# apache/bifromq

Hardware: AMD Instinct MI355X
Metric: publish-topic matches/sec (whole node) (higher is better)
Workload: dtype u32

## Files before the change

bifromq_amd/csrc/bmq_expand_kernel.h:

```cpp
#pragma once

namespace bmq {

constexpr uint32_t SORT_PAIRS = 32;
#ifndef BMQ_EXP_K
#define BMQ_EXP_K 256
#endif
#ifndef BMQ_EXP_LONG
#define BMQ_EXP_LONG 64
#endif
#ifndef BMQ_EXP_CLOCKS
#define BMQ_EXP_CLOCKS 0
#endif
#ifndef BMQ_EXP_MIN_WAVES
#define BMQ_EXP_MIN_WAVES 6
#endif
constexpr uint32_t EXP_K = BMQ_EXP_K;
constexpr uint32_t EXP_LONG = BMQ_EXP_LONG;
constexpr uint32_t EXP_EPL = EXP_K / 64;
constexpr uint32_t EXP_FLAG_WORDS = (EXP_K * (EXP_LONG - 1) + 63) / 64 + 2;
static_assert(EXP_K % 64 == 0 && EXP_K >= 2 * SORT_PAIRS && EXP_K * (EXP_LONG - 1) < 65536, "short-range space: sums are packed into 16 bits below");

#ifndef BMQ_WAVE_EMU
__device__ __forceinline__ uint32_t read_lane(uint32_t v, uint32_t l) { return __builtin_amdgcn_readlane(v, l); }
template <int CTRL, int ROWS> __device__ __forceinline__ uint32_t dpp_take(uint32_t v) {
    return (uint32_t)__builtin_amdgcn_update_dpp(0, (int)v, CTRL, ROWS, 0xF, false);
}
__device__ __forceinline__ uint32_t lane_bit(unsigned long long m) { return (uint32_t)(m >> threadIdx.x) & 1u; }
__device__ __forceinline__ uint32_t first_bit(unsigned long long m) { return (uint32_t)__ffsll((long long)m) - 1u; }
__device__ __forceinline__ uint32_t count_bits(unsigned long long m) { return (uint32_t)__popcll(m); }
__device__ __forceinline__ uint32_t copy_here(uint32_t v) {
    uint32_t r;
    asm volatile("v_mov_b32 %0, %1" : "=v"(r) : "v"(v));
    return r;
}
__device__ __forceinline__ uint32_t uniform_word(const uint32_t* p) { return *scalar_words(p); }
#endif
__device__ __forceinline__ unsigned long long sgpr64(unsigned long long v) {
    return ((unsigned long long)sgpr((uint32_t)(v >> 32)) << 32) | sgpr((uint32_t)v);
}
__device__ __forceinline__ uint32_t wave_incl_scan(uint32_t v) {
    v += dpp_take<0x111, 0xF>(v);
    v += dpp_take<0x112, 0xF>(v);
    v += dpp_take<0x114, 0xF>(v);
    v += dpp_take<0x118, 0xF>(v);
    v += dpp_take<0x142, 0xA>(v);
    v += dpp_take<0x143, 0xC>(v);
    return v;
}
template <int CTRL, int ROWS> __device__ __forceinline__ unsigned long long dpp_take64(unsigned long long v) {
    return ((unsigned long long)dpp_take<CTRL, ROWS>((uint32_t)(v >> 32)) << 32) | dpp_take<CTRL, ROWS>((uint32_t)v);
}
__device__ __forceinline__ unsigned long long wave_total_u64(unsigned long long v) {
    v += dpp_take64<0x111, 0xF>(v);
    v += dpp_take64<0x112, 0xF>(v);
    v += dpp_take64<0x114, 0xF>(v);
    v += dpp_take64<0x118, 0xF>(v);
    v += dpp_take64<0x142, 0xA>(v);
    v += dpp_take64<0x143, 0xC>(v);
    return ((unsigned long long)read_lane((uint32_t)(v >> 32), 63) << 32) | read_lane((uint32_t)v, 63);
}

__device__ __forceinline__ void expand_wave(const BatchArgs& a, const uint32_t block_x, const uint32_t r0 = 0u, const uint32_t r1 = 64u) {
    __shared__ uint32_t s_begin[EXP_K], s_cnt[EXP_K];
    __shared__ uint32_t s_delta[EXP_K + 4];
    __shared__ unsigned long long s_flag[EXP_FLAG_WORDS];
    __shared__ unsigned long long s_rs[2][EXP_EPL];
    __shared__ unsigned long long s_rows[1];
    __shared__ uint32_t s_ind[EXP_K / 32];
    __shared__ uint32_t l_po[64], l_px[65];
    __shared__ uint8_t nz[64];
    uint32_t* const s_key = s_delta;
    const uint32_t lane = threadIdx.x;
    const uint32_t blk = block_x;
    if (blk >= a.n_blocks) return;
    const uint32_t t = (blk << a.tpw_shift) + lane;
    const bool valid = lane < (1u << a.tpw_shift) && t < a.n_topics;
    const bool dbg_x = BMQ_EXP_CLOCKS && BMQ_DBG(a, 4u) && a.dbg_wave;
    const unsigned long long xc0 = dbg_x ? __builtin_amdgcn_s_memtime() : 0ull;
    unsigned long long xc_load = 0, xc_scan = 0, xc_gen = 0;
    const uint32_t status = uniform_word(&a.ctr->status);
    const uint32_t tt = valid ? t : 0u;
    uint32_t nr = a.route_cnt[tt], po = a.pair_off[tt], np = a.pair_cnt[tt];
    unsigned long long acc = 0;
    {
        const uint32_t sb = blk >> SUPER_SHIFT, w0 = sb << SUPER_SHIFT;
        const unsigned long long s0 = a.super_sums[(size_t)min(lane, sb) * SUPER_STRIDE];
        unsigned long long w[4];
#pragma unroll
        for (uint32_t j = 0; j < 4; j++) w[j] = a.wave_sums[min(w0 + lane + 64u * j, blk)];
        static_assert(SUPER_SHIFT == 8, "four loads per lane cover a super-block");
        for (uint32_t i = lane + 64u; i < sb; i += 64) acc += a.super_sums[(size_t)i * SUPER_STRIDE];
        if (lane < sb) acc += s0;
#pragma unroll
        for (uint32_t j = 0; j < 4; j++)
            if (w0 + lane + 64u * j < blk) acc += w[j];
    }
    if (!valid) nr = 0u, po = 0u, np = 0u;
    const bool mine = lane >= r0 && lane < r1;
    if (!mine) np = 0u;
    if (r0 == 0u && a.blk_stats && ((blk & ((1u << SUPER_SHIFT) - 1u)) == (1u << SUPER_SHIFT) - 1u || blk == a.n_blocks - 1)) {
        unsigned long long v = 0, r = 0, b = 0;
        for (uint32_t i = ((blk >> SUPER_SHIFT) << SUPER_SHIFT) + lane; i <= blk; i += 64) {
            const uint4 q = a.blk_stats[i];
            v += q.x, r += q.y, b += q.z;
        }
        v = wave_total_u64(v), r = wave_total_u64(r), b = wave_total_u64(b);
        if (lane == 0) {
            if (v) atomicAdd(&a.ctr->n_visit, v);
            if (r) atomicAdd(&a.ctr->n_ranges, r);
            if (b) atomicAdd(&a.ctr->topic_bytes, b);
        }
    }
    const uint32_t nr_incl = wave_incl_scan(nr);
    const uint32_t wtotal = read_lane(nr_incl, 63);
    const unsigned long long wbase = wave_total_u64(acc);
    const unsigned long long row = wbase + (nr_incl - nr);
    const unsigned long long wend = wbase + wtotal;
    const bool range_err = wend >= 0xFFFFFFFFull, no_space = wend > a.out_capacity;
    if (blk == a.n_blocks - 1 && lane == 0 && r0 == 0u) {
        a.ctr->total_ids = wend;
        *a.out_total = wend;
    }
    if ((range_err || no_space) && lane == 0) atomicOr(&a.ctr->status, range_err ? (uint32_t)ST_RANGE : (uint32_t)ST_NOSPACE);
    const bool writable = !(status & ST_RERUN) && !range_err && !no_space;
    if (valid && mine && !range_err) {
        a.out_row_ptr[t] = (uint32_t)row;
        if (t == a.n_topics - 1) a.out_row_ptr[a.n_topics] = (uint32_t)(row + nr);
    }
    if (!writable || wtotal == 0) return;
    const uint32_t np_incl = wave_incl_scan(np);
    const uint32_t ptotal = read_lane(np_incl, 63);
    if (ptotal == 0) return;
    const uint32_t pexcl = np_incl - np;
    const unsigned long long m_np = ballot64(np != 0);
    const uint32_t first_l = m_np ? first_bit(m_np) : 0u;
    const uint32_t po0 = read_lane(po, first_l) - read_lane(pexcl, first_l);
    const bool contiguous = ballot64(np != 0 && po != po0 + pexcl) == 0ull && !BMQ_DBG(a, 64u);
    l_po[lane] = po;
    l_px[lane] = pexcl;
    if (lane == 63) l_px[64] = ptotal;
    if (np) nz[rank_below(m_np)] = (uint8_t)lane;
    for (uint32_t i = lane; i < EXP_FLAG_WORDS; i += 64) s_flag[i] = 0ull;
    if (lane < EXP_K / 32) s_ind[lane] = 0u;
    if (lane == 0) s_rows[0] = 0ull;
    wave_sync();
    struct Pass {
        uint32_t kn;
        uint32_t ord0;
        uint32_t continues;
    };
    auto plan = [&](uint32_t k0, unsigned long long* rs) -> Pass {
        Pass p;
        p.kn = min(EXP_K, ptotal - k0);
        {
            const uint32_t kend = k0 + p.kn;
            const unsigned long long m = ballot64(pexcl < kend && kend < pexcl + np && np <= SORT_PAIRS);
            if (m) p.kn = read_lane(pexcl, first_bit(m)) - k0;
        }
        const uint32_t lo = pexcl > k0 ? pexcl : k0, hi = min(pexcl + np, k0 + p.kn);
        if (lane < EXP_EPL) rs[lane] = 0ull;
        wave_sync();
        if (lo < hi) atomicOr(&rs[(lo - k0) >> 6], 1ull << ((lo - k0) & 63u));
        const unsigned long long m_k0 = ballot64(np != 0 && pexcl <= k0 && k0 < pexcl + np);
        const uint32_t lk = first_bit(m_k0);
        p.ord0 = count_bits(m_np & ((1ull << lk) - 1ull));
        p.continues = read_lane(pexcl, lk) < k0 ? 1u : 0u;
        wave_sync();
        return p;
    };
    MatchRange pf[EXP_EPL];
    auto fetch = [&](uint32_t k0, const Pass& p, const unsigned long long* rs) {
        const uint32_t lane = lane_here();
        if (contiguous) {
#pragma unroll
            for (uint32_t i = 0; i < EXP_EPL; i++) pf[i] = a.pairs[po0 + k0 + min(lane + 64 * i, p.kn - 1u)];
        } else {
            uint32_t c = p.ord0 - 1u;
            uint32_t at[EXP_EPL];
            const uint32_t l0 = nz[p.ord0];
            const uint32_t at0 = l_po[l0] + (k0 - l_px[l0]);
#pragma unroll
            for (uint32_t i = 0; i < EXP_EPL; i++) {
                const unsigned long long w = sgpr64(rs[i]);
                const uint32_t e = lane + 64 * i;
                at[i] = at0;
                if (e < p.kn) {
                    const uint32_t l = nz[c + rank_below(w) + lane_bit(w)];
                    at[i] = l_po[l] + (k0 + e - l_px[l]);
                }
                c += count_bits(w);
            }
#pragma unroll
            for (uint32_t i = 0; i < EXP_EPL; i++) pf[i] = a.pairs[at[i]];
        }
    };
#pragma unroll
    for (uint32_t i = 0; i < EXP_EPL; i++) pf[i] = MatchRange{0u, 0u};
    Pass cur = plan(0u, s_rs[0]);
    fetch(0u, cur, s_rs[0]);
    uint32_t eb[EXP_EPL], ec[EXP_EPL];
    __builtin_amdgcn_s_waitcnt(0x0F70);
#pragma unroll
    for (uint32_t i = 0; i < EXP_EPL; i++) eb[i] = copy_here(pf[i].begin), ec[i] = copy_here(pf[i].count);
    const unsigned long long xc1 = dbg_x ? __builtin_amdgcn_s_memtime() : 0ull;
    uint32_t pass = 0;
    unsigned long long out_done = read_lane(nr_incl - nr, r0);
    uint32_t carry_last = 0;
    for (uint32_t k0 = 0; k0 < ptotal; pass++) {
        const unsigned long long xp0 = dbg_x ? __builtin_amdgcn_s_memtime() : 0ull;
        const uint32_t kn = cur.kn;
        const bool continues = cur.continues != 0u;
        const unsigned long long* rs = s_rs[pass & 1u];
        unsigned long long rsw[EXP_EPL];
        uint32_t rsc[EXP_EPL];
        {
            uint32_t c = cur.ord0 - 1u;
#pragma unroll
            for (uint32_t i = 0; i < EXP_EPL; i++) {
                rsw[i] = sgpr64(rs[i]);
                rsc[i] = c;
                c += count_bits(rsw[i]);
            }
        }
        unsigned long long m_ind = 0;
#pragma unroll
        for (uint32_t i = 0; i < EXP_EPL; i++) m_ind |= ballot64(lane + 64 * i < kn && (ec[i] & RANGE_INDIRECT) != 0u);
        const bool more = k0 + kn < ptotal;
        Pass nxt = cur;
        if (more) {
            nxt = plan(k0 + kn, s_rs[(pass + 1u) & 1u]);
            fetch(k0 + kn, nxt, s_rs[(pass + 1u) & 1u]);
        }
        auto body = [&](auto ind_tag) {
            constexpr bool IND = decltype(ind_tag)::value;
            auto first_id = [&](uint32_t b, uint32_t cf) -> uint32_t { return (IND && (cf & RANGE_INDIRECT)) ? a.ix.route_pos[b] : b; };
            auto last_id = [&](uint32_t b, uint32_t cf) -> uint32_t {
                const uint32_t c = cf & ~RANGE_INDIRECT;
                return (IND && (cf & RANGE_INDIRECT)) ? a.ix.route_pos[b + c - 1u] : b + c - 1u;
            };
            uint32_t ek[EXP_EPL];
#pragma unroll
            for (uint32_t i = 0; i < EXP_EPL; i++) {
                const uint32_t e = lane + 64 * i;
                ek[i] = eb[i];
                if (e < kn) {
                    ek[i] = first_id(eb[i], ec[i]);
                    s_begin[e] = eb[i];
                    s_cnt[e] = ec[i];
                    s_key[e] = ek[i];
                }
            }
            wave_sync();
            unsigned long long any_bad = 0;
#pragma unroll
            for (uint32_t i = 0; i < EXP_EPL; i++) {
                const uint32_t e = lane + 64 * i;
                bool bad = false;
                if (e < kn && (e == 0u ? continues : lane_bit(rsw[i]) == 0u)) {
                    const uint32_t plast = e == 0u ? carry_last : last_id(s_begin[e - 1u], s_cnt[e - 1u]);
                    bad = ek[i] <= plast;
                }
                any_bad |= ballot64(bad);
            }
            if (any_bad) {
                uint32_t to[EXP_EPL];
#pragma unroll
                for (uint32_t i = 0; i < EXP_EPL; i++) {
                    const uint32_t e = lane + 64 * i;
                    to[i] = e;
                    if (e < kn) {
                        const uint32_t l = nz[rsc[i] + rank_below(rsw[i]) + lane_bit(rsw[i])];
                        const uint32_t s0 = l_px[l], n = l_px[l + 1u] - s0;
                        if (n > 1u && n <= SORT_PAIRS) {
                            const uint32_t first = s0 - k0;
                            const unsigned long long mine = ((unsigned long long)ek[i] << 32) | e;
                            uint32_t rank = 0;
                            const uint32_t end = first + n;
#pragma nounroll
                            for (uint32_t j = first; j < end; j += 4) {
                                const uint32_t q0 = s_key[j], q1 = s_key[j + 1u], q2 = s_key[j + 2u], q3 = s_key[j + 3u];
                                rank += ((((unsigned long long)q0) << 32) | j) < mine ? 1u : 0u;
                                rank += (j + 1u < end && ((((unsigned long long)q1) << 32) | (j + 1u)) < mine) ? 1u : 0u;
                                rank += (j + 2u < end && ((((unsigned long long)q2) << 32) | (j + 2u)) < mine) ? 1u : 0u;
                                rank += (j + 3u < end && ((((unsigned long long)q3) << 32) | (j + 3u)) < mine) ? 1u : 0u;
                            }
                            to[i] = first + rank;
                        }
                    }
                }
                wave_sync();
#pragma unroll
                for (uint32_t i = 0; i < EXP_EPL; i++)
                    if (lane + 64 * i < kn) {
                        s_begin[to[i]] = eb[i];
                        s_cnt[to[i]] = ec[i];
                        s_key[to[i]] = ek[i];
                    }
                wave_sync();
#pragma unroll
                for (uint32_t i = 0; i < EXP_EPL; i++) {
                    const uint32_t e = lane + 64 * i;
                    if (e < kn && (e == 0u ? continues : lane_bit(rsw[i]) == 0u)) {
                        const uint32_t plast = e == 0u ? carry_last : last_id(s_begin[e - 1u], s_cnt[e - 1u]);
                        if (s_key[e] <= plast) {
                            const uint32_t l = nz[rsc[i] + rank_below(rsw[i]) + lane_bit(rsw[i])];
                            atomicOr(&s_rows[0], 1ull << l);
                        }
                    }
                }
            }
            carry_last = sgpr(last_id(s_begin[kn - 1u], s_cnt[kn - 1u]));
            wave_sync();
            const unsigned long long xp1 = dbg_x ? __builtin_amdgcn_s_memtime() : 0ull;
            uint32_t T, stot;
            {
                uint32_t pb[EXP_EPL], pc[EXP_EPL];
                uint32_t s = 0, ss = 0;
                const uint32_t e0 = lane * EXP_EPL;
#pragma unroll
                for (uint32_t i = 0; i < EXP_EPL; i++) {
                    const uint32_t e = e0 + i;
                    pb[i] = e < kn ? s_begin[e] : 0u;
                    pc[i] = e < kn ? s_cnt[e] : 0u;
                    const uint32_t len = pc[i] & ~RANGE_INDIRECT;
                    s += len;
                    if (len - 1u < EXP_LONG - 1u) ss += len + (1u << 16);
                }
                const uint32_t s_incl = wave_incl_scan(s), ss_incl = wave_incl_scan(ss);
                T = read_lane(s_incl, 63);
                stot = read_lane(ss_incl, 63);
                uint32_t run = s_incl - s;
                uint32_t us = (ss_incl - ss) & 0xFFFFu, ord = (ss_incl - ss) >> 16;
#pragma unroll
                for (uint32_t i = 0; i < EXP_EPL; i++) {
                    const uint32_t e = e0 + i;
                    if (e < kn) {
                        const uint32_t len = pc[i] & ~RANGE_INDIRECT;
                        if (len - 1u < EXP_LONG - 1u) {
                            s_delta[ord] = pb[i] - us;
                            if (IND && (pc[i] & RANGE_INDIRECT)) atomicOr(&s_ind[ord >> 5], 1u << (ord & 31u));
                            us += len;
                            atomicOr(&s_flag[(us - 1u) >> 6], 1ull << ((us - 1u) & 63u));
                            ord++;
                        } else s_delta[EXP_K - 1u - (e - ord)] = run;
                        run += len;
                    }
                }
            }
            wave_sync();
            const unsigned long long xp2 = dbg_x ? __builtin_amdgcn_s_memtime() : 0ull;
            __builtin_amdgcn_s_waitcnt(0x0F70);
#pragma unroll
            for (uint32_t i = 0; i < EXP_EPL; i++) eb[i] = copy_here(pf[i].begin), ec[i] = copy_here(pf[i].count);
            {
                uint32_t* const out = a.out_ids + wbase + out_done;
                const bool other = (stot >> 16) != kn;
                uint32_t outp = 0;
                uint32_t ub = 0;
                uint32_t lq = 0;
                uint32_t fw = 0, fo = 0;
                unsigned long long fm = sgpr64(s_flag[0]), fnext = sgpr64(s_flag[1]);
                for (uint32_t k = 0; k < kn;) {
                    uint32_t kl = kn;
                    if (other)
                        for (uint32_t c0 = k; c0 < kn && kl == kn; c0 += 64) {
                            const unsigned long long m = ballot64(c0 + lane < kn && (s_cnt[c0 + lane] & ~RANGE_INDIRECT) - 1u >= EXP_LONG - 1u);
                            if (m) kl = c0 + first_bit(m);
                        }
                    const uint32_t run_end = kl < kn ? sgpr(s_delta[EXP_K - 1u - lq]) : T;
                    if (run_end != outp) {
                        const uint32_t ue = ub + (run_end - outp);
                        uint32_t* const dst = out + outp;
                        for (uint32_t c = ub & ~63u; c < ue; c += 64) {
                            if (fw < (c >> 6)) {
                                fo += count_bits(fm);
                                fw++;
                                fm = fnext;
                                fnext = sgpr64(s_flag[min(fw + 1u, EXP_FLAG_WORDS - 1u)]);
                            }
                            const uint32_t u = c + lane;
                            if (u >= ub && u < ue) {
                                const uint32_t o = fo + rank_below(fm);
                                uint32_t v = s_delta[o] + u;
                                if (IND && ((s_ind[o >> 5] >> (o & 31u)) & 1u)) v = a.ix.route_pos[v];
                                dst[u - ub] = v;
                            }
                        }
                        ub = ue;
                    }
                    if (kl < kn) {
                        const uint32_t b = sgpr(s_begin[kl]), cf = sgpr(s_cnt[kl]), c = cf & ~RANGE_INDIRECT;
                        uint32_t* const dst = out + run_end;
                        if (IND && (cf & RANGE_INDIRECT)) {
                            for (uint32_t o = lane; o < c; o += 64) dst[o] = a.ix.route_pos[b + o];
                        } else {
                            const uint32_t head = min((uint32_t)(((16u - ((uintptr_t)dst & 15u)) & 15u) >> 2), c);
                            if (lane < head) dst[lane] = b + lane;
                            uint4* d4 = reinterpret_cast<uint4*>(dst + head);
                            const uint32_t n4 = (c - head) >> 2;
                            for (uint32_t q = lane; q < n4; q += 64) {
                                const uint32_t v = b + head + 4 * q;
                                d4[q] = make_uint4(v, v + 1, v + 2, v + 3);
                            }
                            for (uint32_t o = head + 4 * n4 + lane; o < c; o += 64) dst[o] = b + o;
                        }
                        outp = run_end + c;
                        lq++;
                    }
                    k = kl + 1;
                }
            }
            out_done += T;
            if (more) {
                wave_sync();
                for (uint32_t i = lane; i <= ((stot & 0xFFFFu) >> 6); i += 64) s_flag[i] = 0ull;
                if (IND && lane < EXP_K / 32 && lane <= (stot >> 21)) s_ind[lane] = 0u;
                wave_sync();
            }
            if (dbg_x) {
                const unsigned long long xp3 = __builtin_amdgcn_s_memtime();
                xc_load += xp1 - xp0, xc_scan += xp2 - xp1, xc_gen += xp3 - xp2;
            }
        };
        if (m_ind) body(std::true_type{});
        else body(std::false_type{});
        k0 += kn;
        cur = nxt;
    }
    if (dbg_x && lane == 0) a.dbg_wave[blk] = make_uint4((uint32_t)(xc1 - xc0), (uint32_t)xc_load, (uint32_t)xc_scan, (uint32_t)xc_gen);
    wave_sync();
    if (valid && lane_bit(s_rows[0]) && nr > 1) {
        const uint32_t sp = atomicAdd(&a.ctr->sort_count, 1u);
        if (sp < a.sort_cap) a.sort_list[sp] = t;
        else atomicOr(&a.ctr->status, ST_NEED_SORTLIST);
    }
}

__global__ __launch_bounds__(64, BMQ_EXP_MIN_WAVES) void k_expand(BatchArgs a) {
    uint32_t bx = blockIdx.x;
    if (a.heavy_list == nullptr) return expand_wave(a, bx);
    constexpr uint32_t HP = EXPAND_PARTS - 1u, RP = 64u / EXPAND_PARTS;
    const uint32_t n_help = HP * a.heavy_cap;
    if (bx < n_help) {
        const uint32_t listed = min(uniform_word(&a.ctr->heavy_count), a.heavy_cap);
        const uint32_t h = bx / HP, part = 1u + bx % HP;
        if (h >= listed) return;
        return expand_wave(a, uniform_word(&a.heavy_list[h]), part * RP, (part + 1u) * RP);
    }
    bx -= n_help;
    if (bx >= a.n_blocks) return;
    const bool split = uniform_word(reinterpret_cast<const uint32_t*>(a.blk_stats + bx) + 3) != 0u;
    expand_wave(a, bx, 0u, split ? RP : 64u);
}

}
```

Measured before the change: 3.994 billion.

## Compact sort to flagged groups and prefetch next flag-chunk delta lookups

After: 4.041 billion, median of 6. +1.2%, better.

```diff
diff --git a/bifromq_amd/csrc/bmq_expand_kernel.h b/bifromq_amd/csrc/bmq_expand_kernel.h
--- a/bifromq_amd/csrc/bmq_expand_kernel.h
+++ b/bifromq_amd/csrc/bmq_expand_kernel.h
@@ -20,6 +20,28 @@
 constexpr uint32_t EXP_EPL = EXP_K / 64;
 constexpr uint32_t EXP_FLAG_WORDS = (EXP_K * (EXP_LONG - 1) + 63) / 64 + 2;
 static_assert(EXP_K % 64 == 0 && EXP_K >= 2 * SORT_PAIRS && EXP_K * (EXP_LONG - 1) < 65536, "short-range space: sums are packed into 16 bits below");
+constexpr uint32_t EXP_IDX_BITS = EXP_K <= 256 ? 8u : 16u;
+using exp_idx_t = std::conditional_t<(EXP_K <= 256), uint16_t, uint32_t>;
+
+#ifdef BMQ_WAVE_EMU
+struct ExpandCoverage {
+    unsigned long long passes = 0, fast_passes = 0;
+    unsigned long long sort_passes = 0;
+    unsigned long long sort_entries = 0, sort_groups = 0;
+    unsigned long long groups[EXP_EPL + 1] = {};
+    unsigned long long unsortable = 0;
+    unsigned long long interleaved = 0;
+    unsigned long long carry_bad = 0;
+    unsigned long long chunks = 0, chunks_held = 0;
+    unsigned long long chunks_ahead = 0;
+};
+inline ExpandCoverage expand_cov;
+#define BMQ_EXP_COV(stmt) do { if (threadIdx.x == 0) { stmt; } } while (0)
+#define BMQ_EXP_COV_ANY(stmt) do { stmt; } while (0)
+#else
+#define BMQ_EXP_COV_ANY(stmt) do { } while (0)
+#define BMQ_EXP_COV(stmt) do { } while (0)
+#endif
 
 #ifndef BMQ_WAVE_EMU
 __device__ __forceinline__ uint32_t read_lane(uint32_t v, uint32_t l) { return __builtin_amdgcn_readlane(v, l); }
@@ -67,6 +89,8 @@
     __shared__ unsigned long long s_flag[EXP_FLAG_WORDS];
     __shared__ unsigned long long s_rs[2][EXP_EPL];
     __shared__ unsigned long long s_rows[1];
+    __shared__ unsigned long long s_need[1];
+    __shared__ exp_idx_t s_idx[EXP_K];
     __shared__ uint32_t s_ind[EXP_K / 32];
     __shared__ uint32_t l_po[64], l_px[65];
     __shared__ uint8_t nz[64];
@@ -143,7 +167,7 @@
     if (np) nz[rank_below(m_np)] = (uint8_t)lane;
     for (uint32_t i = lane; i < EXP_FLAG_WORDS; i += 64) s_flag[i] = 0ull;
     if (lane < EXP_K / 32) s_ind[lane] = 0u;
-    if (lane == 0) s_rows[0] = 0ull;
+    if (lane == 0) s_rows[0] = 0ull, s_need[0] = 0ull;
     wave_sync();
     struct Pass {
         uint32_t kn;
@@ -234,6 +258,7 @@
         }
         auto body = [&](auto ind_tag) {
             constexpr bool IND = decltype(ind_tag)::value;
+            const uint32_t lane = lane_here();
             auto first_id = [&](uint32_t b, uint32_t cf) -> uint32_t { return (IND && (cf & RANGE_INDIRECT)) ? a.ix.route_pos[b] : b; };
             auto last_id = [&](uint32_t b, uint32_t cf) -> uint32_t {
                 const uint32_t c = cf & ~RANGE_INDIRECT;
@@ -253,6 +278,7 @@
             }
             wave_sync();
             unsigned long long any_bad = 0;
+            BMQ_EXP_COV(expand_cov.passes++);
 #pragma unroll
             for (uint32_t i = 0; i < EXP_EPL; i++) {
                 const uint32_t e = lane + 64 * i;
@@ -260,21 +286,48 @@
                 if (e < kn && (e == 0u ? continues : lane_bit(rsw[i]) == 0u)) {
                     const uint32_t plast = e == 0u ? carry_last : last_id(s_begin[e - 1u], s_cnt[e - 1u]);
                     bad = ek[i] <= plast;
+                    if (bad) {
+                        const uint32_t ord = rsc[i] + rank_below(rsw[i]) + lane_bit(rsw[i]);
+                        const uint32_t l = nz[ord];
+                        if (l_px[l + 1u] - l_px[l] <= SORT_PAIRS) atomicOr(&s_need[0], 1ull << ord);
+                        else atomicOr(&s_rows[0], 1ull << l);
+#ifdef BMQ_WAVE_EMU
+                        if (l_px[l + 1u] - l_px[l] > SORT_PAIRS) expand_cov.unsortable++;
+                        if (e == 0u) expand_cov.carry_bad++;
+#endif
+                    }
                 }
                 any_bad |= ballot64(bad);
             }
+            if (!any_bad) BMQ_EXP_COV(expand_cov.fast_passes++);
             if (any_bad) {
-                uint32_t to[EXP_EPL];
-#pragma unroll
-                for (uint32_t i = 0; i < EXP_EPL; i++) {
-                    const uint32_t e = lane + 64 * i;
-                    to[i] = e;
-                    if (e < kn) {
-                        const uint32_t l = nz[rsc[i] + rank_below(rsw[i]) + lane_bit(rsw[i])];
-                        const uint32_t s0 = l_px[l], n = l_px[l + 1u] - s0;
-                        if (n > 1u && n <= SORT_PAIRS) {
+                wave_sync();
+                const unsigned long long need = sgpr64(s_need[0]);
+                if (need) {
+                    uint32_t nb = 0;
+#pragma unroll
+                    for (uint32_t i = 0; i < EXP_EPL; i++) {
+                        const uint32_t e = lane + 64 * i;
+                        const uint32_t ord = rsc[i] + rank_below(rsw[i]) + lane_bit(rsw[i]);
+                        const bool sel = e < kn && ((need >> (ord & 63u)) & 1ull) != 0ull;
+                        const unsigned long long m = ballot64(sel);
+                        if (sel) s_idx[nb + rank_below(m)] = (exp_idx_t)(e | (ord << EXP_IDX_BITS));
+                        nb += count_bits(m);
+                    }
+                    if (lane == 0) s_need[0] = 0ull;
+                    wave_sync();
+                    BMQ_EXP_COV(expand_cov.sort_passes++; expand_cov.sort_entries += nb; expand_cov.sort_groups += (nb + 63u) / 64u; expand_cov.groups[(nb + 63u) / 64u]++);
+#pragma nounroll
+                    for (uint32_t g = (nb + 63u) / 64u; g-- != 0u;) {
+                        const uint32_t c = lane + 64 * g;
+                        uint32_t e = 0, place = 0;
+                        if (c < nb) {
+                            const uint32_t w = s_idx[c];
+                            e = w & ((1u << EXP_IDX_BITS) - 1u);
+                            const uint32_t l = nz[w >> EXP_IDX_BITS];
+                            const uint32_t s0 = l_px[l], n = l_px[l + 1u] - s0;
                             const uint32_t first = s0 - k0;
-                            const unsigned long long mine = ((unsigned long long)ek[i] << 32) | e;
+                            const unsigned long long mine = ((unsigned long long)s_key[e] << 32) | e;
                             uint32_t rank = 0;
                             const uint32_t end = first + n;
 #pragma nounroll
@@ -285,27 +338,34 @@
                                 rank += (j + 2u < end && ((((unsigned long long)q2) << 32) | (j + 2u)) < mine) ? 1u : 0u;
                                 rank += (j + 3u < end && ((((unsigned long long)q3) << 32) | (j + 3u)) < mine) ? 1u : 0u;
                             }
-                            to[i] = first + rank;
+                            place = first + rank;
                         }
-                    }
-                }
-                wave_sync();
-#pragma unroll
-                for (uint32_t i = 0; i < EXP_EPL; i++)
-                    if (lane + 64 * i < kn) {
-                        s_begin[to[i]] = eb[i];
-                        s_cnt[to[i]] = ec[i];
-                        s_key[to[i]] = ek[i];
-                    }
-                wave_sync();
-#pragma unroll
-                for (uint32_t i = 0; i < EXP_EPL; i++) {
-                    const uint32_t e = lane + 64 * i;
-                    if (e < kn && (e == 0u ? continues : lane_bit(rsw[i]) == 0u)) {
-                        const uint32_t plast = e == 0u ? carry_last : last_id(s_begin[e - 1u], s_cnt[e - 1u]);
-                        if (s_key[e] <= plast) {
-                            const uint32_t l = nz[rsc[i] + rank_below(rsw[i]) + lane_bit(rsw[i])];
-                            atomicOr(&s_rows[0], 1ull << l);
+                        wave_sync();
+                        if (c < nb) s_idx[e] = (exp_idx_t)place;
+                    }
+                    wave_sync();
+#pragma unroll
+                    for (uint32_t i = 0; i < EXP_EPL; i++) {
+                        const uint32_t e = lane + 64 * i;
+                        const uint32_t ord = rsc[i] + rank_below(rsw[i]) + lane_bit(rsw[i]);
+                        if (e < kn && ((need >> (ord & 63u)) & 1ull) != 0ull) {
+                            const uint32_t to = s_idx[e];
+                            s_begin[to] = eb[i];
+                            s_cnt[to] = ec[i];
+                            s_key[to] = ek[i];
+                        }
+                    }
+                    wave_sync();
+#pragma unroll
+                    for (uint32_t i = 0; i < EXP_EPL; i++) {
+                        const uint32_t e = lane + 64 * i;
+                        const uint32_t ord = rsc[i] + rank_below(rsw[i]) + lane_bit(rsw[i]);
+                        if (e < kn && lane_bit(rsw[i]) == 0u && ((need >> (ord & 63u)) & 1ull) != 0ull) {
+                            const uint32_t plast = last_id(s_begin[e - 1u], s_cnt[e - 1u]);
+                            if (s_key[e] <= plast) {
+                                atomicOr(&s_rows[0], 1ull << nz[ord]);
+                                BMQ_EXP_COV_ANY(expand_cov.interleaved++);
+                            }
                         }
                     }
                 }
@@ -361,6 +421,14 @@
                 uint32_t lq = 0;
                 uint32_t fw = 0, fo = 0;
                 unsigned long long fm = sgpr64(s_flag[0]), fnext = sgpr64(s_flag[1]);
+                uint32_t oc = rank_below(fm), on = count_bits(fm) + rank_below(fnext);
+                auto ask_ind = [&](uint32_t o) -> uint32_t { return IND ? s_ind[min(o, EXP_K - 1u) >> 5] : 0u; };
+                uint32_t dc = copy_here(s_delta[oc]), ic = IND ? copy_here(ask_ind(oc)) : 0u;
+                unsigned long long fraw = s_flag[min(2u, EXP_FLAG_WORDS - 1u)];
+                uint32_t dn = s_delta[on], in = ask_ind(on);
+#ifdef BMQ_WAVE_EMU
+                uint32_t cov_c = ~0u;
+#endif
                 for (uint32_t k = 0; k < kn;) {
                     uint32_t kl = kn;
                     if (other)
@@ -373,17 +441,24 @@
                         const uint32_t ue = ub + (run_end - outp);
                         uint32_t* const dst = out + outp;
                         for (uint32_t c = ub & ~63u; c < ue; c += 64) {
+#ifdef BMQ_WAVE_EMU
+                            BMQ_EXP_COV(expand_cov.chunks++; if (fw < (c >> 6)) expand_cov.chunks_ahead++; else if (c == cov_c) expand_cov.chunks_held++);
+                            cov_c = c;
+#endif
                             if (fw < (c >> 6)) {
                                 fo += count_bits(fm);
                                 fw++;
                                 fm = fnext;
-                                fnext = sgpr64(s_flag[min(fw + 1u, EXP_FLAG_WORDS - 1u)]);
+                                fnext = sgpr64(((unsigned long long)copy_here((uint32_t)(fraw >> 32)) << 32) | copy_here((uint32_t)fraw));
+                                oc = on, dc = copy_here(dn), ic = IND ? copy_here(in) : 0u;
+                                on = fo + count_bits(fm) + rank_below(fnext);
+                                fraw = s_flag[min(fw + 2u, EXP_FLAG_WORDS - 1u)];
+                                dn = s_delta[on], in = ask_ind(on);
                             }
                             const uint32_t u = c + lane;
                             if (u >= ub && u < ue) {
-                                const uint32_t o = fo + rank_below(fm);
-                                uint32_t v = s_delta[o] + u;
-                                if (IND && ((s_ind[o >> 5] >> (o & 31u)) & 1u)) v = a.ix.route_pos[v];
+                                uint32_t v = dc + u;
+                                if (IND && ((ic >> (oc & 31u)) & 1u)) v = a.ix.route_pos[v];
                                 dst[u - ub] = v;
                             }
                         }
```
